# privefl/bigsnpr

Measured on AMD Instinct MI355X. Metric: SNP-cols/sec for bed_randomSVD k=20 (m*passes/wall), higher is better.
Workload: dtype i8 (2-bit codes x 24-bit (early block steps) / 16-bit (late block steps) fixed-point image of the fp64 basis in int8 slices, exact int32 MFMA accumulation; fp64 panel algebra and Rayleigh-Ritz)

## Files before the change

### bigsnpr_amd/_lib.py

```python
import ctypes as C
import os
import threading

import numpy as np

_HERE = os.path.dirname(os.path.abspath(__file__))
LIB_PATH = os.path.join(_HERE, "libbigsnpr_hip.so")

u8p = C.POINTER(C.c_uint8)
i32p = C.POINTER(C.c_int32)
i64p = C.POINTER(C.c_int64)
u64p = C.POINTER(C.c_uint64)
f64p = C.POINTER(C.c_double)
vp = C.c_void_p
i64 = C.c_int64

ALLREDUCE_FN = C.CFUNCTYPE(None, C.c_void_p, C.c_int64, C.c_void_p)


class SvdOptions(C.Structure):
    _fields_ = [("k", C.c_int32), ("tol", C.c_double), ("block", C.c_int32),
                ("slices", C.c_int32), ("max_basis", C.c_int32), ("seed", C.c_uint32),
                ("verbose", C.c_int32), ("m_total", C.c_int64), ("allreduce", ALLREDUCE_FN),
                ("allreduce_ctx", C.c_void_p), ("hook_rank", C.c_int32), ("hook_world", C.c_int32),
# ... 84 lines not shown
    "bsn_bed_project_pca": (C.c_int, [vp, i64p, i64, i64p, i64, f64p, f64p, f64p, i64, f64p, f64p, f64p, f64p]),
    "bsn_project_last_ms": (C.c_int, [f64p]),
    "bsn_mult_lin_reg":(C.c_int, [vp, i64p, i64, i64p, i64, f64p, i64, f64p]),
    "bsn_univ_linreg": (C.c_int, [vp, i64p, i64, i64p, i64, f64p, f64p, i64, f64p, f64p]),
    "bsn_univ_logreg": (C.c_int, [vp, i64p, i64, i64p, i64, f64p, f64p, i64, C.c_double, C.c_int32, f64p, f64p, i32p]),
    "bsn_bed_sp_reg": (C.c_int, [vp, i64p, i64, i64p, i64] + _PLR_TAIL),
    "bsn_dense_sp_reg": (C.c_int, [vp, C.c_int, i64, i64, i64] + _PLR_TAIL),
    "bsn_plr_last_stats": (C.c_int, [f64p]),
    "bsn_impute_simple": (C.c_int, [vp, C.c_int, C.c_uint64, C.POINTER(vp), u8p, i64p]),
    "bsn_impute_last_ms": (C.c_int, [f64p]),
    "bsn_inflate": (C.c_int, [u8p, i64p, i64, u8p, i64p, i32p]),
    "bsn_bgen_read": (C.c_int, [C.c_char_p, i64p, i64, i64, i64p, i64, u8p, C.c_int, C.c_uint64, i64, i64, i64, C.POINTER(vp), u8p,
                                f64p, f64p]),
    "bsn_bgen_prod": (C.c_int, [C.c_char_p, i64p, i64, i64, i64p, i64, f64p, C.c_int, C.c_uint64, i64, f64p, i64, i64, i64, f64p]),
    "bsn_bgen_last_ms": (C.c_int, [f64p]),
    "bsn_bed_group_counts": (C.c_int, [vp, i64p, i64, i32p, C.c_int32, i64p, i64, i32p]),
    "bsn_fst": (C.c_int, [f64p, f64p, i64, i64, C.c_double, f64p, f64p]),
    "bsn_bed_fst": (C.c_int, [vp, i64p, i64, i32p, C.c_int32, i64p, i64, C.c_double, f64p, f64p]),
    "bsn_snp_max3": (C.c_int, [vp, i64p, i64, i32p, i64p, i64, f64p, C.c_int32, f64p]),
    "bsn_popstat_last_ms": (C.c_int, [f64p]),
    "bsn_hwe": (C.c_int, [i32p, i64, C.c_int, f64p]),
    "bsn_hwe_lanes": (C.c_int, [i32p, i64, C.c_int, C.c_int, f64p, f64p]),
    "bsn_bed_hwe": (C.c_int, [vp, i64p, i64, i64p, i64, C.c_int, f64p, i32p]),
    "bsn_bed_qc": (C.c_int, [vp, i64p, i64, i64p, i64, i32p, C.c_double, C.c_double, C.c_double, C.c_double, C.c_int,
                             u8p, u8p, f64p, f64p]),
    "bsn_qc_last_ms": (C.c_int, [f64p]),
    "bsn_bed_king": (C.c_int, [vp, i64p, i64, i64p, i64, C.c_double, C.c_int, C.POINTER(C.c_int64), C.POINTER(vp)]),
    "bsn_king_fetch": (C.c_int, [vp, i32p, i32p, i32p, f64p]),
    "bsn_king_free": (C.c_int, [vp]),
    "bsn_king_last_ms": (C.c_int, [f64p]),
    "bsn_bed_to_fbm": (C.c_int, [vp, i64p, i64, i64p, i64, u8p]),
    "bsn_bed_readbina": (C.c_int, [vp, u8p, u8p]),
    "bsn_bed_is_streamed": (C.c_int, [vp]),
    "bsn_bed_streaming_kernels": (C.c_int, [vp, C.c_char_p, i64]),
    "bsn_bed_subset_payload": (C.c_int, [vp, i64p, i64, i64p, i64, u8p]),
    "bsn_op_create": (C.c_int, [vp, i64p, i64, i64p, i64, f64p, f64p, C.POINTER(vp)]),
    "bsn_op_destroy": (C.c_int, [vp]),
    "bsn_op_set_slices": (C.c_int, [vp, C.c_int]),
    "bsn_op_prod": (C.c_int, [vp, vp, i64, C.c_int, vp, i64]),
    "bsn_op_cprod": (C.c_int, [vp, vp, i64, C.c_int, vp, i64]),
    "bsn_op_sync": (C.c_int, [vp]),
    "bsn_op_last_kernel": (C.c_int, [vp, C.c_char_p, i64]),
    "bsn_bed_randomsvd": (C.c_int, [vp, i64p, i64, i64p, i64, f64p, f64p, C.POINTER(SvdOptions),
                                    f64p, f64p, f64p, C.POINTER(SvdInfo)]),
    "bsn_bed_tcrossprod": (C.c_int, [vp, i64p, i64, i64p, i64, f64p, f64p, i64, f64p]),
    "bsn_cormat": (C.c_int, [vp, i64p, i64, i64p, i64, C.c_double, f64p, f64p, C.c_int, i32p,
                             C.POINTER(C.c_int64), C.POINTER(vp)]),
    "bsn_cormat_fetch": (C.c_int, [vp, i32p, f64p]),
    "bsn_cormat_has_nan": (C.c_int, [vp, C.POINTER(C.c_int)]),
    "bsn_cormat_free": (C.c_int, [vp]),
    "bsn_ld_scores": (C.c_int, [vp, i64p, i64, i64p, i64, C.c_double, f64p, f64p]),
    "bsn_clumping_chr": (C.c_int, [vp, i64p, i64, i64p, i64, C.c_int, f64p, f64p, i32p, i32p, f64p,
                                   C.c_double, C.c_double, i32p]),
    "bsn_clumping_chr_cached": (C.c_int, [vp, i64p, i64, i64p, i64, C.c_int, f64p, f64p, i32p, i32p, f64p,
                                          i64, f64p, f64p, i32p]),
    "bsn_snp_grid_prs": (C.c_int, [vp, i64p, i64, i64p, i64, f64p, i32p, C.POINTER(C.c_uint8), i64, i64,
                                   C.c_int, f64p]),
    "bsn_sfbm_from_csc": (C.c_int, [i64p, i32p, f64p, i64, C.c_int, C.POINTER(vp)]),
    "bsn_sfbm_ncol": (C.c_int, [vp, i64p, i64p, i64p]),
    "bsn_sfbm_free": (C.c_int, [vp]),
    "bsn_lassosum2": (C.c_int, [vp, f64p, i64, f64p, f64p, f64p, i64, i64p, C.c_double, C.c_int32, C.c_double,
                                f64p, i32p, f64p]),
    "bsn_ldpred2_gibbs": (C.c_int, [vp, f64p, f64p, i64, i64p, f64p, f64p, i32p, u64p, i64, C.c_int, C.c_int, C.c_uint64,
                                    f64p, f64p]),
    "bsn_ldpred2_gibbs_sampling": (C.c_int, [vp, f64p, f64p, i64, i64p, C.c_double, C.c_double, C.c_int32, C.c_uint64,
                                             C.c_int, C.c_int, C.c_uint64, f64p, f64p]),
    "bsn_ldpred2_auto": (C.c_int, [vp, f64p, f64p, f64p, i64, i64p, f64p, u64p, i64, C.c_double, C.c_int, C.c_int, C.c_int,
                                   C.c_int, C.c_double, C.c_int, C.c_double, C.c_double, C.c_double, C.c_double,
                                   C.c_double, C.c_uint64, f64p, f64p, f64p, f64p, f64p, f64p, f64p, f64p]),
    "bsn_sfbm_prodvec": (C.c_int, [vp, f64p, i64p, i64, f64p]),
    "bsn_sfbm_ld_scores": (C.c_int, [vp, i64p, i64, f64p]),
    "bsn_sfbm_solve_sym": (C.c_int, [vp, f64p, f64p, i64p, i64, C.c_double, C.c_int32, f64p, i32p, f64p]),
    "bsn_sfbm_last_ms": (C.c_int, [vp, f64p]),
    "bsn_sfbm_ldsplit": (C.c_int, [vp, C.c_double, C.c_double, C.c_int32, C.c_int32, C.c_int32, C.c_double, f64p, f64p, i32p,
                                   f64p, f64p, f64p, i32p, i32p, i32p, f64p]),
    "bsn_panel_gemm_tn": (C.c_int, [vp, i64, C.c_int32, vp, i64, C.c_int32, i64, vp, C.c_int32]),
    "bsn_panel_gemm_nn": (C.c_int, [vp, i64, C.c_int32, vp, C.c_int32, vp, i64, C.c_double, C.c_double, vp, i64, i64]),
    "bsn_panel_right_mult": (C.c_int, [vp, i64, i64, C.c_int32, C.c_int32, vp]),
    "bsn_panel_update": (C.c_int, [vp, i64, C.c_int32, vp, vp, C.c_int32, vp, i64, i64, vp]),
    "bsn_panel_round_cols": (C.c_int, [vp, i64, i64, C.c_int32, C.c_int32, C.c_int32, vp, C.c_int32]),
    "bsn_panel_fused_orth": (C.c_int, [vp, i64, C.c_int32, C.c_int32, C.c_int32, C.c_int32, f64p, f64p]),
    "bsn_panel_compact_gather": (C.c_int, [vp, i64, C.c_int32, C.c_int32, C.c_int32, vp]),
    "bsn_panel_block_roundtrip": (C.c_int, [vp, i64, C.c_int32, C.c_int32, vp, vp]),
    "bsn_malloc": (C.c_int, [C.POINTER(vp), i64]),
    "bsn_free": (C.c_int, [vp]),
    "bsn_host_alloc": (C.c_int, [C.POINTER(vp), i64]),
    "bsn_host_free": (C.c_int, [vp]),
    "bsn_memcpy_h2d": (C.c_int, [vp, vp, i64]),
    "bsn_memcpy_d2h": (C.c_int, [vp, vp, i64]),
    "bsn_device_sync": (C.c_int, []),
    "bsn_timer_start": (C.c_int, [vp]),
    "bsn_timer_stop": (C.c_int, [vp, f64p]),
}

_lib = None


class BsnError(RuntimeError):
    pass


def load():
    global _lib
    if _lib is None:
        LIB_PATH = os.environ.get("BSN_LIB_PATH") or globals()["LIB_PATH"]
        if not os.path.exists(LIB_PATH):
            raise ImportError(
                "%s not found: build it with `python -m bigsnpr_amd.build` "
                "(there is no CPU fallback)" % LIB_PATH)
        lib = C.CDLL(LIB_PATH)
        for name, (res, args) in SIGNATURES.items():
            fn = getattr(lib, name)
            fn.restype = res
            fn.argtypes = args
        _lib = lib
    return _lib


def check(rc):
    if rc != 0:
        raise BsnError(load().bsn_last_error().decode("utf-8", "replace"))


def ptr(a, t):
    return None if a is None else a.ctypes.data_as(t)


def as_i64(a):
    return None if a is None else np.ascontiguousarray(a, dtype=np.int64)


def as_f64(a):
    return None if a is None else np.ascontiguousarray(a, dtype=np.float64)


class DeviceArray:

    def __init__(self, rows, cols=1):
        self.rows, self.cols = int(rows), int(cols)
        p = vp()
        check(load().bsn_malloc(C.byref(p), self.rows * self.cols * 8))
        self.ptr = p

    @classmethod
    def from_numpy(cls, a):
        a = np.asarray(a, dtype=np.float64)
        if a.ndim == 1:
            a = a[:, None]
        d = cls(a.shape[0], a.shape[1])
        h = np.asfortranarray(a)
        check(load().bsn_memcpy_h2d(d.ptr, h.ctypes.data_as(vp), h.nbytes))
        return d

    def to_numpy(self):
        h = np.empty((self.rows, self.cols), dtype=np.float64, order="F")
        check(load().bsn_memcpy_d2h(h.ctypes.data_as(vp), self.ptr, h.nbytes))
        return h

    def col_ptr(self, j):
        return vp(self.ptr.value + 8 * self.rows * j)

    def free(self):
        if self.ptr is not None and self.ptr.value:
            load().bsn_free(self.ptr)
            self.ptr = None

    def __del__(self):
        try:
            self.free()
        except Exception:
            pass


class _PinnedBlock:

    def __init__(self, pool, addr, size):
        self.pool, self.addr, self.size = pool, addr, size
        self.__array_interface__ = {"data": (addr, False), "shape": (size,), "typestr": "|u1", "version": 3}

    def __del__(self):
        try:
            self.pool._give_back(self.addr, self.size)
        except Exception:
            pass


class PinnedPool:

    def __init__(self, keep=None):
        self.free = []
        self.keep = int(os.environ.get("BSN_RESULT_POOL_KEEP", 1 << 30)) if keep is None else keep
        self.keep_max = int(os.environ.get("BSN_RESULT_POOL_MAX", 8 << 30))
        self.live = 0
        self.peak_live = 0
# ... 77 lines not shown
```

### bigsnpr_amd/csrc/matvec.hip

```cpp
#include <cmath>
#include <cstdlib>
#include <map>
#include <mutex>

#include "bsn_internal.hpp"
#include "byte_plan.hpp"
#include "prod_plan.hpp"
#include "prodt_sparse.hpp"
#include <type_traits>

namespace bsn {

typedef int v4i __attribute__((ext_vector_type(4)));
typedef int v8i __attribute__((ext_vector_type(8)));

static thread_local const void *g_last_kernel = nullptr;
#define BSN_KLAUNCH(kern, ...)                 \
  do {                                         \
    g_last_kernel = (const void *)(kern);      \
    hipLaunchKernelGGL(kern, __VA_ARGS__);     \
  } while (0)

__device__ __forceinline__ uint32_t lut4(uint32_t lut, uint32_t sel) {
  return __builtin_amdgcn_perm(lut, lut, sel);
// ... 117 lines not shown
  if (blockIdx.x == 0 && tid == 0) meta[v].qscale = qs;
  double xa[16], xc[16], xs[16];
#pragma unroll
  for (int it = 0; it < 16; it++) {
    const int64_t k = (int64_t)blockIdx.x * 1024 + it * 64 + tid;
    const bool in = k < len;
    xa[it] = in ? X[k + v * ldx] : 0.0;
    xc[it] = 0.0;
    xs[it] = 1.0;
    if (mode == 1) {
      if (in && scale) xs[it] = scale[k];
      if (in && center) xc[it] = center[k];
    } else if (mode == 2) {
      if (in && center) xc[it] = center[k + v * ldx];
    }
  }
#pragma unroll
  for (int it = 0; it < 16; it++) {
    const int t = it * 64 + tid;
    double a = xa[it], b = 0;
    if (mode == 1) {
      a = a / xs[it];
      b = (xc[it] - voff) * a;
      a *= vstep;
    } else if (mode == 2) {
      b = xc[it];
    }
    if (!(fabs(a) <= 1.79e308)) a = 0;
    if (!(fabs(b) <= 1.79e308)) b = 0;
    sa[t + (t >> 4)] = a * qs;
    sb[t + (t >> 4)] = b * qs;
  }
  __syncthreads();
  long long shi = 0, slo = 0, shi2 = 0, slo2 = 0;
  if (kb * 16 < len_pad) {
    uint32_t pk[2][S][4];
#pragma unroll
    for (int p = 0; p < 2; p++)
#pragma unroll
      for (int s = 0; s < S; s++)
#pragma unroll
        for (int w = 0; w < 4; w++) pk[p][s][w] = 0;
#pragma unroll
    for (int e = 0; e < 16; e++) {
      long long A = llrint(sa[tid * 17 + e]), B = llrint(sb[tid * 17 + e]);
      shi += A >> 24; slo += A & 0xFFFFFF;
      shi2 += B >> 24; slo2 += B & 0xFFFFFF;
      if ((raw3 & 1) && PERM != 2) B -= 3 * A;
      const int pos = PERM == 1 ? ((e & 3) * 4 + (e >> 2)) : e;
#pragma unroll
      for (int s = 0; s < S; s++) {
        const int8_t da = (int8_t)(A & 0xFF), db = (int8_t)(B & 0xFF);
        A = (A - da) >> 8;
        B = (B - db) >> 8;
        if constexpr (PERM == 2) {
          const int r = prodt_sparse_row(e), ba = prodt_sparse_byte(e, 0), bb = prodt_sparse_byte(e, 1);
          pk[r][s][ba >> 2] |= (uint32_t)(uint8_t)da << (8 * (ba & 3));
          pk[r][s][bb >> 2] |= (uint32_t)(uint8_t)db << (8 * (bb & 3));
        } else {
          pk[0][s][pos >> 2] |= (uint32_t)(uint8_t)da << (8 * (pos & 3));
          pk[1][s][pos >> 2] |= (uint32_t)(uint8_t)db << (8 * (pos & 3));
        }
      }
    }
    for (int p = 0; p < nplanes; p++)
#pragma unroll
      for (int s = 0; s < S; s++) {
        const int col = v * S + s;
        int8_t *dst = q + ((kb * nplanes + p) * ncol + col) * 16;
        *(uint4 *)dst = p == 0 ? uint4{pk[0][s][0], pk[0][s][1], pk[0][s][2], pk[0][s][3]}
                               : uint4{pk[1][s][0], pk[1][s][1], pk[1][s][2], pk[1][s][3]};
      }
  }
  for (int off = 32; off > 0; off >>= 1) {
    shi += __shfl_down(shi, off); slo += __shfl_down(slo, off);
    shi2 += __shfl_down(shi2, off); slo2 += __shfl_down(slo2, off);
  }
  if (tid == 0) {
    atomicAdd((unsigned long long *)&meta[v].sum_hi, (unsigned long long)shi);
    atomicAdd((unsigned long long *)&meta[v].sum_lo, (unsigned long long)slo);
    if (mode >= 1) {
      atomicAdd((unsigned long long *)&meta[v].sum2_hi, (unsigned long long)shi2);
      atomicAdd((unsigned long long *)&meta[v].sum2_lo, (unsigned long long)slo2);
    }
  }
}

template <int NB, int NPLANE, int KC, bool RAW0, bool STATS, bool CONTIG, int TILES = 2, int WAVES = 8, int MINW = 1,
          int TAG = 0, bool TILED = false, int SGB = 0, bool NASKIP = false>
__global__ __launch_bounds__(64 * WAVES, MINW) void k_cprod(const uint8_t *__restrict__ img, int64_t pitch,
                                               const int32_t *__restrict__ cols, int64_t col0,
                                               int64_t m, const int8_t *__restrict__ xq,
                                               int32_t *__restrict__ acc_out, int64_t m_out,
                                               uint32_t lutA, uint32_t lutB, uint32_t lutC,
                                               int32_t *__restrict__ counts, int32_t n_pad_samples,
                                               const CprodGrid geo, int32_t *__restrict__ part_out) {
  constexpr int NCOL = 16 * NB;
  constexpr int LD = KC / 256;
  constexpr int XS = KC / 16 * NCOL;
  __shared__ uint4 xs[2][XS];
  const int tid = threadIdx.x, wave = tid >> 6, lane = tid & 63;
  const int c = lane & 15, g = lane >> 4;
  constexpr int NT = 64 * WAVES;
  const int nchunks = (int)(pitch * 4 / KC);
  constexpr bool GEO = CONTIG && !TILED && !STATS && NPLANE < 3 && KC == 512;
  CprodSlab sl{(int)blockIdx.x, 0, 0, nchunks};
  if constexpr (GEO) {
    sl = cprod_slab(geo, blockIdx.x);
    sl.block = __builtin_amdgcn_readfirstlane(sl.block), sl.slab = __builtin_amdgcn_readfirstlane(sl.slab);
    sl.ch_begin = __builtin_amdgcn_readfirstlane(sl.ch_begin), sl.ch_end = __builtin_amdgcn_readfirstlane(sl.ch_end);
  }
  const int ch_begin = sl.ch_begin, ch_end = sl.ch_end;
  if (ch_begin >= ch_end) return;
  const int64_t wg_base = (int64_t)sl.block * (WAVES * 16 * TILES);
  const int64_t snp_base = wg_base + wave * (16 * TILES);
  const uint8_t *rowp[TILES];
  uint32_t voff[TILES];
#pragma unroll
  for (int t = 0; t < TILES; t++) {
    int64_t j = snp_base + t * 16 + c;
    if (j > m - 1) j = m - 1;
    int64_t col = CONTIG ? col0 + j : (int64_t)cols[j];
    rowp[t] = img + col * pitch + g * 16;
    voff[t] = TILED ? (uint32_t)((((j - wg_base) >> 6) * (pitch >> 8)) * 16384 + (j & 63) * 256 + g * 16)
                    : (uint32_t)((j - wg_base) * pitch + g * 16);
  }
  static_assert(!TILED || (CONTIG && (WAVES * 16 * TILES) % 64 == 0), "streaming layout: whole 64-variant blocks");
  const __amdgpu_buffer_rsrc_t rs = __builtin_amdgcn_make_buffer_rsrc(
      (void *)(TILED ? img + (((col0 + wg_base) >> 6) * (pitch >> 8)) * 16384
                     : img + (col0 + (CONTIG ? wg_base : 0)) * pitch),
      0, 0x7fffffff, 0x00020000);
  typedef unsigned int v4u __attribute__((ext_vector_type(4)));
  auto gload = [&](const int t, const int off) -> uint4 {
    if constexpr (CONTIG) {
      const int soff = TILED ? ((off >> 8) << 14) + (off & 255) : off;
      const v4u r = __builtin_amdgcn_raw_buffer_load_b128(rs, (int)voff[t], soff, 0);
      return uint4{r.x, r.y, r.z, r.w};
    } else {
      return *(const uint4 *)(rowp[t] + off);
    }
  };
  const uint4 *xq4 = (const uint4 *)xq;

  v4i acc[TILES][NPLANE][NB];
#pragma unroll
  for (int t = 0; t < TILES; t++)
#pragma unroll
    for (int p = 0; p < NPLANE; p++)
#pragma unroll
      for (int nb = 0; nb < NB; nb++) acc[t][p][nb] = v4i{0, 0, 0, 0};
  uint32_t st_lo[TILES], st_hi[TILES], st_na[TILES];
#pragma unroll
  for (int t = 0; t < TILES; t++) st_lo[t] = st_hi[t] = st_na[t] = 0;

  constexpr int NX = (XS + NT - 1) / NT;
  static_assert(NX <= 4, "staging registers");
  constexpr bool XFULL = (XS % NT == 0);
  uint4 ga[2][TILES][LD];
  uint4 xr0 = {0, 0, 0, 0}, xr1 = {0, 0, 0, 0}, xr2 = {0, 0, 0, 0}, xr3 = {0, 0, 0, 0};
#pragma unroll
  for (int t = 0; t < TILES; t++)
#pragma unroll
    for (int it = 0; it < LD; it++) ga[0][t][it] = gload(t, ch_begin * (KC / 4) + it * 64);
  auto staged = [&](const int x) -> bool { return XFULL || tid + x * NT < XS; };
  {
    const uint4 *src = xq4 + (int64_t)ch_begin * XS;
// ... 785 lines not shown
    load(jn2, X[SET]);
#pragma unroll
    for (int q = 0; q < 4; q++) {
      v4i val, na;
      if constexpr (HASNA) {
        uint32_t n0, n1, n2, n3;
        val = v4i{(int)val8m(T[q][0], n0), (int)val8m(T[q][1], n1), (int)val8m(T[q][2], n2), (int)val8m(T[q][3], n3)};
        na = v4i{(int)n0, (int)n1, (int)n2, (int)n3};
      } else {
        val = v4i{(int)T[q][0], (int)T[q][1], (int)T[q][2], (int)T[q][3]};
      }
#pragma unroll
      for (int nb = 0; nb < NB; nb++) {
        acc[q][nb] = __builtin_amdgcn_mfma_i32_16x16x64_i8(aw[nb], val, acc[q][nb], 0, 0, 0);
        if constexpr (HASNA) acc[q][nb] = __builtin_amdgcn_mfma_i32_16x16x64_i8(awc[nb], na, acc[q][nb], 0, 0, 0);
      }
    }
    ws[SET ^ 1][wtid] = wreg;
    __syncthreads();
  };
  for (int64_t jb = j0; jb < j1; jb += 128) {
    step(std::integral_constant<int, 0>{}, jb);
    if (jb + 64 < j1) step(std::integral_constant<int, 1>{}, jb + 64);
  }
  if (wbase < n_pad) {
#pragma unroll
    for (int u = 0; u < 4; u++) {
      const int64_t i = wbase + sg * 4 + u;
#pragma unroll
      for (int nb = 0; nb < NB; nb++)
        *(v4i *)(acc_out + (((int64_t)blockIdx.y * n_pad + i) * NCOL + nb * 16 + 4 * g)) = acc[u][nb];
    }
  }
}

void require_bits(const bsn_bed *b, int bits, const char *what) {
  if (b->bits != bits)
    fail("%s is not available for this handle: it needs %s", what,
         bits == 2 ? "a 2-bit genotype image (.bed, or an FBM.code256 whose codes decode to 0 / 1 / 2 / NA)"
                   : "a byte (dosage) image");
}

void prof_begin(bsn_op *op, int kind, bool more) {
  if (!op->profile) return;
  if (op->prof_kind_override >= 0) kind = op->prof_kind_override;
  op->ev_more.push_back(more);
  hipEvent_t a, b;
  BSN_HIP(hipEventCreate(&a));
  BSN_HIP(hipEventCreate(&b));
  op->ev_begin.push_back(a);
  op->ev_end.push_back(b);
  op->ev_kind.push_back(kind);
  BSN_HIP(hipEventRecord(a, op->bed->stream));
}
void prof_end(bsn_op *op) {
  if (!op->profile) return;
  BSN_HIP(hipEventRecord(op->ev_end.back(), op->bed->stream));
  op->prof_kernel[op->ev_kind.back() % kProfKinds] = g_last_kernel;
}
void prof_collect(bsn_op *op, double ms[kProfKinds], int count[kProfKinds]) {
  for (int k = 0; k < kProfKinds; k++) ms[k] = 0, count[k] = 0;
  for (size_t i = 0; i < op->ev_begin.size(); i++) {
    float t = 0;
    if (hipEventSynchronize(op->ev_end[i]) == hipSuccess &&
        hipEventElapsedTime(&t, op->ev_begin[i], op->ev_end[i]) == hipSuccess) {
      ms[op->ev_kind[i]] += t;
      if (!op->ev_more[i]) count[op->ev_kind[i]]++;
    }
    (void)hipEventDestroy(op->ev_begin[i]);
    (void)hipEventDestroy(op->ev_end[i]);
  }
  (void)hipGetLastError();
  op->ev_begin.clear();
  op->ev_end.clear();
  op->ev_kind.clear();
  op->ev_more.clear();
}

static VecMeta *meta_buffer(bsn_op *op) {
  return (VecMeta *)op->d_meta.ensure((size_t)kMetaVecs * 8 + (size_t)kMetaVecs * 256 * 2);
}
static inline int64_t n_padded(const bsn_bed *b) { return b->bits == 8 ? b->pitch : b->pitch * 4; }

static void quantise(bsn_op *op, const double *d_X, int64_t ldx, int64_t len, int64_t len_pad,
                     int nvec, int mode, int S, int ncol, int permute, int exact_int,
                     VecMeta *meta, int8_t *q, const double *d_W2 = nullptr) {
  hipStream_t st = op->bed->stream;
  const bool bytes = op->bed->bits == 8;
  const double vstep = bytes ? op->bed->v_step : 1.0, voff = bytes ? op->bed->v_off : 0.0;
  const int raw3 = (!bytes && mode == 1) ? 1 : 0;
  if (bytes) permute = 0;
  if (permute == 2 && !(mode == 1 && (raw3 & 1))) fail("internal: the interleaved digit rows are the scaled product's");
  double *part = (double *)(meta + kMetaVecs);
  int gx = 0;
  if (exact_int) {
    hipLaunchKernelGGL(k_meta_clear, dim3(1), dim3(64), 0, st, meta, nvec);
  } else {
    gx = (int)((len + 1023) / 1024);
    if (gx > 256) gx = 256;
    hipLaunchKernelGGL(k_absmax, dim3(gx, nvec), dim3(1024), 0, st, d_X, ldx, len,
                       mode == 1 ? op->d_center.p : mode == 2 ? d_W2 : nullptr,
                       mode == 1 ? op->d_scale.p : nullptr, mode, meta, part, vstep, voff, raw3);
  }
  int64_t nblk = len_pad / 16;
  const double *qc = mode == 1 ? op->d_center.p : mode == 2 ? d_W2 : nullptr;
  const double *qsc = mode == 1 ? op->d_scale.p : nullptr;
  const dim3 qgrid((unsigned)((nblk + 63) / 64), nvec);
#define BSN_QUANT(SV)                                                                                  \
  case SV:                                                                                             \
    if (permute == 2)                                                                                  \
      hipLaunchKernelGGL((k_quant<SV, 2>), qgrid, dim3(64), 0, st, d_X, ldx, len, len_pad, qc, qsc, mode, \
                         ncol, meta, q, vstep, voff, raw3, part, gx);                                  \
    else if (permute)                                                                                  \
      hipLaunchKernelGGL((k_quant<SV, 1>), qgrid, dim3(64), 0, st, d_X, ldx, len, len_pad, qc, qsc, mode, \
                         ncol, meta, q, vstep, voff, raw3, part, gx);                                  \
    else                                                                                               \
      hipLaunchKernelGGL((k_quant<SV, 0>), qgrid, dim3(64), 0, st, d_X, ldx, len, len_pad, qc, qsc, mode, \
                         ncol, meta, q, vstep, voff, raw3, part, gx);                                  \
    break;
  switch (S) {
    BSN_QUANT(1) BSN_QUANT(2) BSN_QUANT(3) BSN_QUANT(4) BSN_QUANT(5) BSN_QUANT(6) BSN_QUANT(7) BSN_QUANT(8)
    default: fail("slices must be in 1..8");
  }
#undef BSN_QUANT
  BSN_HIP(hipGetLastError());
}

static const double *scatter_rows_if_needed(bsn_op *op, const double *d_X, int64_t *ldx,
                                            int nvec) {
  if (op->rows_identity) return d_X;
  bsn_bed *b = op->bed;
  double *xf = op->d_xfull.ensure((size_t)b->n * nvec);
  BSN_HIP(hipMemsetAsync(xf, 0, (size_t)b->n * nvec * sizeof(double), b->stream));
  hipLaunchKernelGGL(k_scatter_rows, dim3((unsigned)((op->n + 255) / 256), nvec), dim3(256), 0,
                     b->stream, d_X, *ldx, op->d_rows.p, op->n, xf, b->n);
  BSN_HIP(hipGetLastError());
  *ldx = b->n;
  return xf;
}

#pragma clang fp contract(off)
__global__ void k_binom_scale(const int32_t *counts, int64_t m, double *center, double *scale) {
  int64_t j = (int64_t)blockIdx.x * blockDim.x + threadIdx.x;
  if (j >= m) return;
  const int4 c = *(const int4 *)(counts + 4 * j);
  const double sumX = (double)(c.y + 2 * c.z);
  const double nona = (double)(c.x + c.y + c.z);
  const double af = sumX / (2.0 * nona);
  center[j] = 2.0 * af;
  scale[j] = sqrt(2.0 * af * (1.0 - af));
}
#pragma clang fp contract(on)

__global__ __launch_bounds__(256) void k_stats_summary(const int32_t *counts, int64_t m, int64_t n, int32_t *na,
                                                       unsigned long long *out) {
  long long s = 0, bad = 0;
  for (int64_t j = (int64_t)blockIdx.x * 256 + threadIdx.x; j < m; j += (int64_t)gridDim.x * 256) {
    const int4 c = *(const int4 *)(counts + 4 * j);
    s += c.w;
    na[j] = c.w;
    if (2 * ((int64_t)c.x + c.y + c.z) < n) bad++;
  }
  for (int off = 32; off > 0; off >>= 1) {
    s += __shfl_down(s, off);
    bad += __shfl_down(bad, off);
  }
  __shared__ long long sw[4], sb[4];
  if ((threadIdx.x & 63) == 0) {
    sw[threadIdx.x >> 6] = s;
    sb[threadIdx.x >> 6] = bad;
  }
  __syncthreads();
  if (threadIdx.x == 0) {
    s = sw[0] + sw[1] + sw[2] + sw[3];
    bad = sb[0] + sb[1] + sb[2] + sb[3];
    if (s) atomicAdd(&out[0], (unsigned long long)s);
    if (bad) atomicAdd(&out[1], (unsigned long long)bad);
  }
}

static bool use_tiled(const bsn_op *op) {
  return op->bed->d_tiled != nullptr && op->cols_contig && (op->col0 & 63) == 0;
}

static int device_cus() {
  static const int ncu = [] {
    hipDeviceProp_t pr;
    int dev = 0;
    return (hipGetDevice(&dev) == hipSuccess && hipGetDeviceProperties(&pr, dev) == hipSuccess && pr.multiProcessorCount > 0)
               ? pr.multiProcessorCount : 256;
  }();
  return ncu;
}

static thread_local CprodGridFacts g_cprod_facts;
static CprodGrid cprod_geometry(bsn_op *op, const void *kern, int per_wg, int threads, int NB, int nplane) {
  static std::mutex mu;
  static std::map<const void *, int> held;
  int resident;
  {
    std::lock_guard<std::mutex> lk(mu);
    auto it = held.find(kern);
    if (it == held.end()) {
      int nb = 0;
      if (hipOccupancyMaxActiveBlocksPerMultiprocessor(&nb, kern, threads, 0) != hipSuccess || nb < 1) nb = 1;
      it = held.emplace(kern, nb).first;
    }
    resident = it->second;
  }
  CprodGridFacts f;
  f.m = op->m, f.per_wg = per_wg, f.nchunks = (int)(op->bed->pitch * 4 / 512), f.pitch = op->bed->pitch;
  f.NB = NB, f.nplane = nplane, f.ncu = device_cus(), f.resident = resident;
  if (const char *e = getenv("BSN_PLAN_CUS")) f.ncu = std::max(1, atoi(e));
  if (const char *e = getenv("BSN_CPROD_SLABS")) f.slabs = std::max(1, atoi(e));
  g_cprod_facts = f;
  return plan_cprod(f);
}

template <int NPLANE, bool RAW0, bool STATS>
static void launch_cprod(bsn_op *op, int NB, const int8_t *q, int32_t *acc, uint32_t l0,
                         uint32_t l1, uint32_t l2, int32_t *counts = nullptr, CprodGrid *geo = nullptr,
                         int32_t *part = nullptr) {
  bsn_bed *b = op->bed;
  constexpr int KC = 512, TT = STATS ? 2 : 4;
  constexpr bool PLAIN = NPLANE == 2 && RAW0 && !STATS;
  if (b->pitch * 4 > 4000000) fail("more than 4e6 samples are not supported by the crossproduct kernel");
  const int32_t *cols = op->cols_contig ? nullptr : op->d_cols.p;
  const int32_t npad = (int32_t)(b->pitch * 4 - b->n);
  CprodFacts f;
  f.NB = NB, f.plain = PLAIN, f.stats = STATS, f.cols_contig = op->cols_contig, f.tiled = use_tiled(op);
  f.warm = op->prof_kind_override == 3, f.na_skip = op->na_skip_c;
  const CprodKernel k = choose_cprod(f);
  const uint8_t *image = k.tiled ? b->d_tiled : b->d_img;
  const int per_wg = 16 * k.tiles * k.waves;
  const bool geo_ok = geo && k.contig && !k.tiled && !STATS && NPLANE < 3 && !getenv("BSN_CPROD_ONE_SPLIT");
  CprodGrid one;
  one.blocks = one.blocks_whole = (int)((op->m + per_wg - 1) / per_wg), one.nchunks = (int)(b->pitch * 4 / KC);
  const bool planning = geo && !acc;
  if (planning && !geo_ok) {
    *geo = one;
    return;
  }
  const CprodGrid g = geo && !planning ? *geo : one;
  const dim3 grid((unsigned)cprod_workgroups(g)), block(64 * k.waves);
#define BSN_CPROD(NBV, CONTIGV, TV, WV, TAGV, TILEDV, SGBV, NASKIPV)                                                   \
  if (k == CprodKernel{NBV, CONTIGV, TV, WV, TAGV, TILEDV, SGBV, NASKIPV}) {                                           \
    auto kern = k_cprod<NBV, NPLANE, KC, RAW0, STATS, CONTIGV, TV, WV, 1, TAGV, TILEDV, SGBV, NASKIPV>;                \
    if (planning) {                                                                                                    \
      *geo = cprod_geometry(op, (const void *)kern, per_wg, 64 * k.waves, NB, NPLANE);                                 \
      return;                                                                                                          \
    }                                                                                                                  \
    BSN_KLAUNCH(kern, grid, block, 0, b->stream, image, b->pitch, cols, op->col0, op->m, q, acc, op->m, l0, l1, l2,    \
                counts, npad, g, part);                                                                                \
    BSN_HIP(hipGetLastError());                                                                                        \
    return;                                                                                                            \
  }
  BSN_CPROD(1, false, 2, 8, 0, false, 0, false)
  BSN_CPROD(1, true, 2, 8, 0, false, 0, false)
  BSN_CPROD(1, true, 2, 8, 1, false, 0, false)
  BSN_CPROD(1, true, TT, 8, 0, true, 0, false)
  BSN_CPROD(1, true, TT, 8, 1, true, 0, false)
  BSN_CPROD(2, false, 2, 16, 0, false, 0, false)
  BSN_CPROD(2, true, 2, 16, 0, false, 3, false)
  BSN_CPROD(2, true, 2, 16, 0, true, 3, false)
  if constexpr (!STATS && NPLANE < 3) {
    BSN_CPROD(3, false, 2, 16, 0, false, 0, false)
    BSN_CPROD(3, true, 2, 16, 0, false, 3, false)
  }
  if constexpr (PLAIN) {
    BSN_CPROD(2, false, 2, 16, 0, false, 0, true)
    BSN_CPROD(2, true, 2, 16, 0, false, 0, true)
    BSN_CPROD(3, false, 2, 16, 0, false, 0, true)
    BSN_CPROD(3, true, 2, 16, 0, false, 0, true)
  }
#undef BSN_CPROD
// ... 558 lines not shown
                    bool one_digit, int32_t *d_table, double ms_out[3]) {
  require_bits(op->bed, 2, "bed_counts_by_group");
  op->preq_X = nullptr;
  bsn_bed *b = op->bed;
  hipStream_t st = b->stream;
  const int S = one_digit ? 1 : 4, per_block = 16 / S;
  const int64_t npad = n_padded(b), nblk = npad / 16;
  const int gmax = G < 2 * per_block ? G : 2 * per_block;
  DevBuf<int32_t> mult;
  mult.ensure((size_t)b->n * gmax);
  int8_t *q = op->d_q.ensure((size_t)npad * 32);
  int32_t *acc = op->d_acc.ensure((size_t)3 * op->m * 32);
  std::unique_ptr<EventMarks<4>> ev(ms_out ? new EventMarks<4>() : nullptr);
  for (int g0 = 0; g0 < G;) {
    const int left = G - g0;
    const int NB = left > per_block ? 2 : 1;
    const int gb = left < NB * per_block ? left : NB * per_block, ncol = 16 * NB;
    if (ev) ev->mark(0, st);
    BSN_HIP(hipMemsetAsync(mult.p, 0, (size_t)b->n * gb * sizeof(int32_t), st));
    hipLaunchKernelGGL(k_group_scatter, dim3((unsigned)((n + 255) / 256)), dim3(256), 0, st, d_rows, d_group, n, g0, gb,
                       b->n, mult.p);
    const dim3 qgrid((unsigned)((nblk + 255) / 256), (unsigned)gb);
    if (S == 1) hipLaunchKernelGGL(k_group_digits<1>, qgrid, dim3(256), 0, st, mult.p, b->n, nblk, gb, ncol, q);
    else hipLaunchKernelGGL(k_group_digits<4>, qgrid, dim3(256), 0, st, mult.p, b->n, nblk, gb, ncol, q);
    BSN_HIP(hipGetLastError());
    if (ev) ev->mark(1, st);
    launch_cprod<3, false, false>(op, NB, q, acc, kLutHom2, kLutHet, kLutNA);
    if (ev) ev->mark(2, st);
    hipLaunchKernelGGL(k_group_counts_final, dim3((unsigned)((op->m * gb + 255) / 256)), dim3(256), 0, st, acc, op->m, ncol,
                       S, g0, gb, G, d_gsize, d_table);
    BSN_HIP(hipGetLastError());
    if (ev) {
      ev->mark(3, st);
      BSN_HIP(hipEventSynchronize(ev->e[3]));
      for (int k = 0; k < 3; k++) ms_out[k] += ev->ms(k, k + 1);
    }
    g0 += gb;
  }
  BSN_HIP(hipStreamSynchronize(st));
}

__global__ void k_selftest(int *out) {
  int lane = threadIdx.x;
  uint32_t r = perm8(0x77665544u, 0x33221100u, 0x07040300u);
  int ok_perm = (r == 0x77443300u);
  v4i a = {0, 0, 0, 0}, b = {0, 0, 0, 0};
  int i = lane & 15, gq = lane >> 4;
  for (int e = 0; e < 16; e++) {
    int k = gq * 16 + e;
    int av = (k == (5 * i + 3) % 64) ? (i + 1) : 0;
    int bv = (k % 7) - 3 + i;
    a[e >> 2] |= (av & 0xFF) << (8 * (e & 3));
    b[e >> 2] |= (bv & 0xFF) << (8 * (e & 3));
  }
  v4i c = {0, 0, 0, 0};
  c = __builtin_amdgcn_mfma_i32_16x16x64_i8(a, b, c, 0, 0, 0);
  int ok_mfma = 1;
  for (int rr = 0; rr < 4; rr++) {
    int row = 4 * gq + rr, col = lane & 15;
    int k = (5 * row + 3) % 64;
    int want = (row + 1) * ((k % 7) - 3 + col);
    if (c[rr] != want) ok_mfma = 0;
  }
  int all_perm = __all(ok_perm), all_mfma = __all(ok_mfma);
  if (lane == 0) {
    out[0] = all_perm;
    out[1] = all_mfma;
    out[2] = (int)r;
  }
}

void selftest() {
  DevBuf<int> d;
  d.ensure(4);
  hipLaunchKernelGGL(k_selftest, dim3(1), dim3(64), 0, 0, d.p);
  BSN_HIP(hipGetLastError());
  int h[4] = {0, 0, 0, 0};
  BSN_HIP(hipMemcpy(h, d.p, sizeof(h), hipMemcpyDeviceToHost));
  if (!h[0]) fail("selftest: v_perm_b32 byte order differs from the assumed {hi:lo} (got %08x)", h[2]);
  if (!h[1]) fail("selftest: v_mfma_i32_16x16x64_i8 operand/accumulator layout differs");
}

}
```

### include/bigsnpr_hip.h

```cpp
#ifndef BIGSNPR_HIP_H
#define BIGSNPR_HIP_H

#include <stdint.h>

#ifdef __cplusplus
extern "C" {
#endif

typedef struct bsn_bed bsn_bed;
typedef struct bsn_op bsn_op;

const char *bsn_last_error(void);
int bsn_version(void);
int bsn_device_count(int *count);
int bsn_set_device(int device);
int bsn_selftest(void);

int bsn_bed_open(const char *path, int64_t n, int64_t m, bsn_bed **out);
int bsn_bed_is_streamed(const bsn_bed *bed);
int bsn_bed_from_host(const uint8_t *payload, int64_t n, int64_t m, int64_t n_byte, bsn_bed **out);
int bsn_bed_from_fbm(const uint8_t *bytes, int64_t n, int64_t m, int64_t ld, bsn_bed **out);
int bsn_fbm_open(const uint8_t *bytes, int64_t n, int64_t m, int64_t ld, const double *code256, bsn_bed **out);
int bsn_bed_bits(const bsn_bed *bed);
int64_t bsn_bed_na_known(const bsn_bed *bed);
// ... 218 lines not shown
int bsn_bed_tcrossprod(bsn_bed *bed, const int64_t *ind_row, int64_t n, const int64_t *ind_col,
                       int64_t m, const double *center, const double *scale, int64_t block_size,
                       double *K);

typedef struct bsn_cor bsn_cor;
int bsn_cormat(bsn_bed *bed, const int64_t *ind_row, int64_t n, const int64_t *ind_col, int64_t m,
               double size, const double *thr, const double *pos, int fill_diag, int32_t *p_out,
               int64_t *nnz_out, bsn_cor **out);
int bsn_cormat_fetch(bsn_cor *cor, int32_t *i_out, double *x_out);
int bsn_cormat_has_nan(const bsn_cor *cor, int *out);
int bsn_cormat_free(bsn_cor *cor);
int bsn_ld_last_stats(double *out );
int bsn_ld_scores(bsn_bed *bed, const int64_t *ind_row, int64_t n, const int64_t *ind_col, int64_t m,
                  double size, const double *pos, double *out);
int bsn_clumping_chr(bsn_bed *bed, const int64_t *ind_row, int64_t n, const int64_t *ind_col,
                     int64_t m, int mode, const double *aux1, const double *aux2,
                     const int32_t *ordInd, const int32_t *rankInd, const double *pos, double size,
                     double thr, int32_t *keep);
int bsn_clumping_chr_cached(bsn_bed *bed, const int64_t *ind_row, int64_t n, const int64_t *ind_col,
                            int64_t m, int mode, const double *aux1, const double *aux2,
                            const int32_t *ordInd, const int32_t *rankInd, const double *pos,
                            int64_t n_grid, const double *sizes, const double *thrs, int32_t *keep);

int bsn_robust_scale_tau2(const double *d_X, int64_t m, int64_t ld, int32_t ncol, double c1, double c2, double *mu_out, double *s_out);
int bsn_robust_medians(const double *d_X, int64_t m, int64_t ld, int32_t ncol, const double *centre, double *med_out);
int bsn_robust_pair_scales(const double *d_Z, int64_t m, int64_t ld, int32_t p, double c1, double c2, double *s_sum_out, double *s_diff_out);
int bsn_robust_mc_count(const double *d_up, int64_t nu, const double *d_lo, int64_t nl, double t, int64_t *count_out);
int bsn_robust_scale_cols(double *d_Z, int64_t m, int64_t ld, int32_t p, const double *div );
int bsn_robust_rotate(double *d_Z, int64_t m, int64_t ld, int32_t p, const double *E );
int bsn_robust_wdist(const double *d_Z, int64_t m, int64_t ld, int32_t p, const double *mu, const double *sig, double *out);
int bsn_robust_dist_ogk(const double *d_U, int64_t m, int64_t ld, int32_t p, int32_t niter, double cut_ratio, double c1, double c2,
                        double *dist_out, int64_t *n_kept_out);
int bsn_robust_rollmean(const double *x, int64_t m, const double *w, int32_t len, const int64_t *group_off, int32_t ngroups, double *out);
int bsn_robust_sort(double *x, int64_t m);
int bsn_robust_mc_window(const double *d_up, int64_t nu, const double *d_lo, int64_t nl, double a, double b, int64_t cap, double *out,
                         int64_t *count_out);

int bsn_order_decreasing(const double *S, int64_t m, const int64_t *group_off, int32_t ngroups, int32_t *ord, int32_t *rank);

typedef struct bsn_sfbm bsn_sfbm;
int bsn_sfbm_from_csc(const int64_t *p, const int32_t *i, const double *x, int64_t m2, int upper, bsn_sfbm **out);
int bsn_sfbm_ncol(const bsn_sfbm *s, int64_t *m2_out, int64_t *nnz_out, int64_t *bandwidth_out);
int bsn_sfbm_free(bsn_sfbm *s);
int bsn_lassosum2(const bsn_sfbm *s, const double *beta_hat, int64_t m, const double *pf, const double *lambda,
                  const double *delta, int64_t G, const int64_t *ind_sub, double dfmax, int32_t maxiter, double tol,
                  double *beta_out, int32_t *num_iter_out, double *time_out);
int bsn_ldpred2_gibbs(const bsn_sfbm *s, const double *beta_hat, const double *n_vec, int64_t m, const int64_t *ind_sub,
                      const double *h2, const double *p, const int32_t *sparse, const uint64_t *stream, int64_t G, int burn_in,
                      int num_iter, uint64_t seed, double *beta_out, double *seconds_out);
int bsn_ldpred2_gibbs_sampling(const bsn_sfbm *s, const double *beta_hat, const double *n_vec, int64_t m, const int64_t *ind_sub,
                               double h2, double p, int32_t sparse, uint64_t stream, int burn_in, int num_iter, uint64_t seed,
                               double *sample_out, double *seconds_out);
int bsn_ldpred2_auto(const bsn_sfbm *s, const double *beta_hat, const double *n_vec, const double *log_var, int64_t m,
                     const int64_t *ind_sub, const double *p_init, const uint64_t *stream, int64_t G, double h2_init,
                     int burn_in, int num_iter, int report_step, int no_jump_sign, double shrink_corr, int use_mle,
                     double p_lo, double p_hi, double alpha_lo, double alpha_hi, double mean_ld, uint64_t seed,
                     double *beta_est, double *postp_est, double *corr_est, double *sample_beta,
                     double *path_p, double *path_h2, double *path_alpha, double *seconds_out);

int bsn_sfbm_prodvec(bsn_sfbm *s, const double *x, const int64_t *ind_sub, int64_t m, double *y_out);
int bsn_sfbm_ld_scores(bsn_sfbm *s, const int64_t *ind_sub, int64_t m, double *out);
int bsn_sfbm_solve_sym(bsn_sfbm *s, const double *b, const double *add_to_diag, const int64_t *ind_sub, int64_t m, double tol,
                       int32_t maxiter, double *x_out, int32_t *iters_out, double *relres_out);
int bsn_sfbm_last_ms(const bsn_sfbm *s, double *ms_out);

int bsn_sfbm_ldsplit(const bsn_sfbm *s, double thr_r2, double max_r2, int32_t min_size, int32_t max_size, int32_t max_K,
                     double max_cost, const double *pos_scaled, double *C_out, int32_t *best_ind_out, double *cost_out,
                     double *cost2_out, double *perc_kept_out, int32_t *n_block_ok_out, int32_t *all_last_out,
                     int32_t *levels_run_out, double *seconds_out);

int bsn_panel_gemm_tn(const double *d_A, int64_t lda, int32_t p, const double *d_B, int64_t ldb, int32_t cb, int64_t rows,
                      double *d_C, int32_t ldc);
int bsn_panel_gemm_nn(const double *d_Q, int64_t ldq, int32_t p, const double *d_S, int32_t nc, const double *d_In, int64_t ldi,
                      double alpha, double beta, double *d_Out, int64_t ldo, int64_t n);
int bsn_panel_right_mult(double *d_W, int64_t ld, int64_t n, int32_t cb, int32_t r, const double *d_M);
int bsn_panel_update(const double *d_Q, int64_t ldq, int32_t p, const double *d_C, const double *d_Ri, int32_t cb, double *d_W,
                     int64_t ldw, int64_t n, uint64_t *d_mx);
int bsn_panel_round_cols(double *d_X, int64_t ld, int64_t rows, int32_t cb, int32_t slices, int32_t have_mx, uint64_t *d_mx,
                         int32_t wide_grid);
int bsn_panel_fused_orth(double *d_QW, int64_t nr, int32_t p, int32_t p0, int32_t cb, int32_t iters, double *flag_out,
                         double *Rout_out);
int bsn_panel_compact_gather(const double *d_full, int64_t n, int32_t cb, int32_t world, int32_t slices, double *d_out);
int bsn_panel_block_roundtrip(const double *d_full, int64_t n, int32_t cb, int32_t world, double *d_out, double *d_placed);

int bsn_malloc(void **d_ptr, int64_t bytes);
int bsn_free(void *d_ptr);
int bsn_host_alloc(void **h_ptr, int64_t bytes);
int bsn_host_free(void *h_ptr);
int bsn_memcpy_h2d(void *d_dst, const void *src, int64_t bytes);
int bsn_memcpy_d2h(void *dst, const void *d_src, int64_t bytes);
int bsn_device_sync(void);
int bsn_timer_start(bsn_bed *bed);
int bsn_timer_stop(bsn_bed *bed, double *ms);

#ifdef __cplusplus
}
#endif
#endif
```

Before: 39.43 million.

## Quantise whole basis panel in one tiled kernel instead of per-vector grids

```diff
diff --git a/bigsnpr_amd/_lib.py b/bigsnpr_amd/_lib.py
--- a/bigsnpr_amd/_lib.py
+++ b/bigsnpr_amd/_lib.py
@@ -190,6 +190,8 @@
     "bsn_panel_fused_orth": (C.c_int, [vp, i64, C.c_int32, C.c_int32, C.c_int32, C.c_int32, f64p, f64p]),
     "bsn_panel_compact_gather": (C.c_int, [vp, i64, C.c_int32, C.c_int32, C.c_int32, vp]),
     "bsn_panel_block_roundtrip": (C.c_int, [vp, i64, C.c_int32, C.c_int32, vp, vp]),
+    "bsn_quant_panel": (C.c_int, [vp, i64, i64, i64, C.c_int32, C.c_int32, C.c_int32, C.c_int32, C.c_int32, vp, vp, C.c_int32,
+                                  C.c_int32, vp, vp]),
     "bsn_malloc": (C.c_int, [C.POINTER(vp), i64]),
     "bsn_free": (C.c_int, [vp]),
     "bsn_host_alloc": (C.c_int, [C.POINTER(vp), i64]),
@@ -218,6 +220,8 @@
                 "(there is no CPU fallback)" % LIB_PATH)
         lib = C.CDLL(LIB_PATH)
         for name, (res, args) in SIGNATURES.items():
+            if name == "bsn_quant_panel" and not hasattr(lib, name):
+                continue
             fn = getattr(lib, name)
             fn.restype = res
             fn.argtypes = args
diff --git a/bigsnpr_amd/csrc/matvec.hip b/bigsnpr_amd/csrc/matvec.hip
--- a/bigsnpr_amd/csrc/matvec.hip
+++ b/bigsnpr_amd/csrc/matvec.hip
@@ -223,6 +223,154 @@
     if (mode >= 1) {
       atomicAdd((unsigned long long *)&meta[v].sum2_hi, (unsigned long long)shi2);
       atomicAdd((unsigned long long *)&meta[v].sum2_lo, (unsigned long long)slo2);
+    }
+  }
+}
+
+constexpr int kQuantTileBlocks = 16;
+constexpr int kQuantTileK = 16 * kQuantTileBlocks;
+constexpr int kQuantPanelVecs = 16;
+template <int S, int PERM>
+__global__ __launch_bounds__(kQuantTileK) void k_quant_panel(const double *__restrict__ X, int64_t ldx, int64_t len,
+                                                             int64_t len_pad, const double *__restrict__ center,
+                                                             const double *__restrict__ scale, int mode, int ncol,
+                                                             int nvec, int tiles, VecMeta *meta, int8_t *__restrict__ q,
+                                                             double vstep, double voff, int raw3,
+                                                             const double *__restrict__ part, int gx) {
+  static_assert(S >= 1 && S <= 3, "the staged integers are int32");
+  constexpr int NT = kQuantTileK, LDW = 17;
+  static_assert(2 * NT * LDW * 4 >= kQuantTileBlocks * 2 * kMaxCols * 16, "the digit rows of a tile fit the value staging");
+  __shared__ uint4 lds4[2 * NT * LDW * 4 / 16];
+  __shared__ double s_qs[kQuantPanelVecs];
+  __shared__ long long s_sum[NT / 64][kQuantPanelVecs][4];
+  int32_t *const sa = (int32_t *)lds4, *const sb = sa + NT * LDW;
+  const int tid = threadIdx.x, wave = tid >> 6, lane = tid & 63;
+  const int nplanes = mode >= 1 ? 2 : 1, nused = nvec * S;
+  for (int v = wave; v < nvec; v += NT / 64) {
+    double mx = 0, bad = 0;
+    for (int t = lane; t < gx; t += 64) {
+      mx = fmax(mx, part[((int64_t)v * gx + t) * 2]);
+      bad += part[((int64_t)v * gx + t) * 2 + 1];
+    }
+    for (int off = 32; off > 0; off >>= 1) {
+      mx = fmax(mx, __shfl_xor(mx, off));
+      bad += __shfl_xor(bad, off);
+    }
+    double qs = 0.0;
+    if (mx > 0) {
+      int e;
+      frexp(ldexp(0.99, 8 * S - 1) / mx, &e);
+      qs = ldexp(1.0, e - 1);
+    }
+    if (lane == 0) {
+      s_qs[v] = qs;
+      if (blockIdx.x == 0) {
+        meta[v].absmax_bits = (unsigned long long)__double_as_longlong(mx);
+        meta[v].nonfinite = (unsigned long long)bad;
+        meta[v].qscale = qs;
+      }
+    }
+  }
+  __syncthreads();
+  const int v2 = tid & 15, kbl = tid >> 4;
+  long long shi = 0, slo = 0, shi2 = 0, slo2 = 0;
+  for (int tile = 0; tile < tiles; tile++) {
+    const int64_t kb0 = ((int64_t)blockIdx.x * tiles + tile) * kQuantTileBlocks;
+    if (kb0 * 16 >= len_pad) break;
+    const int64_t k = kb0 * 16 + tid;
+    const bool in = k < len;
+    double xs = 1.0, xc = 0.0, xa[kQuantPanelVecs];
+    if (mode == 1) {
+      if (in && scale) xs = scale[k];
+      if (in && center) xc = center[k];
+    }
+#pragma unroll
+    for (int v = 0; v < kQuantPanelVecs; v++) xa[v] = (in && v < nvec) ? X[k + v * ldx] : 0.0;
+#pragma unroll
+    for (int v = 0; v < kQuantPanelVecs; v++) {
+      if (v < nvec) {
+        double a = xa[v], b = 0;
+        if (mode == 1) {
+          a = a / xs;
+          b = (xc - voff) * a;
+          a *= vstep;
+        }
+        if (!(fabs(a) <= 1.79e308)) a = 0;
+        if (!(fabs(b) <= 1.79e308)) b = 0;
+        const double qs = s_qs[v];
+        sa[tid * LDW + v] = (int32_t)llrint(a * qs);
+        sb[tid * LDW + v] = (int32_t)llrint(b * qs);
+      }
+    }
+    __syncthreads();
+    uint32_t pk[2][S][4];
+#pragma unroll
+    for (int p = 0; p < 2; p++)
+#pragma unroll
+      for (int s = 0; s < S; s++)
+#pragma unroll
+        for (int w = 0; w < 4; w++) pk[p][s][w] = 0;
+    if (v2 < nvec) {
+#pragma unroll
+      for (int e = 0; e < 16; e++) {
+        long long A = sa[(kbl * 16 + e) * LDW + v2], B = sb[(kbl * 16 + e) * LDW + v2];
+        shi += A >> 24; slo += A & 0xFFFFFF;
+        shi2 += B >> 24; slo2 += B & 0xFFFFFF;
+        if ((raw3 & 1) && PERM != 2) B -= 3 * A;
+        const int pos = PERM == 1 ? ((e & 3) * 4 + (e >> 2)) : e;
+#pragma unroll
+        for (int s = 0; s < S; s++) {
+          const int8_t da = (int8_t)(A & 0xFF), db = (int8_t)(B & 0xFF);
+          A = (A - da) >> 8;
+          B = (B - db) >> 8;
+          if constexpr (PERM == 2) {
+            const int r = prodt_sparse_row(e), ba = prodt_sparse_byte(e, 0), bb = prodt_sparse_byte(e, 1);
+            pk[r][s][ba >> 2] |= (uint32_t)(uint8_t)da << (8 * (ba & 3));
+            pk[r][s][bb >> 2] |= (uint32_t)(uint8_t)db << (8 * (bb & 3));
+          } else {
+            pk[0][s][pos >> 2] |= (uint32_t)(uint8_t)da << (8 * (pos & 3));
+            pk[1][s][pos >> 2] |= (uint32_t)(uint8_t)db << (8 * (pos & 3));
+          }
+        }
+      }
+    }
+    __syncthreads();
+    if (v2 < nvec) {
+      for (int p = 0; p < nplanes; p++)
+#pragma unroll
+        for (int s = 0; s < S; s++)
+          lds4[(kbl * nplanes + p) * nused + v2 * S + s] =
+              p == 0 ? uint4{pk[0][s][0], pk[0][s][1], pk[0][s][2], pk[0][s][3]}
+                     : uint4{pk[1][s][0], pk[1][s][1], pk[1][s][2], pk[1][s][3]};
+    }
+    __syncthreads();
+    int64_t nb = len_pad / 16 - kb0;
+    if (nb > kQuantTileBlocks) nb = kQuantTileBlocks;
+    const int nrows = (int)nb * nplanes * nused;
+    uint4 *const qrow = (uint4 *)q + kb0 * nplanes * ncol;
+    for (int u = tid; u < nrows; u += NT) {
+      const int run = u / nused, c = u - run * nused;
+      qrow[(int64_t)run * ncol + c] = lds4[u];
+    }
+    __syncthreads();
+  }
+  for (int off = 32; off >= 16; off >>= 1) {
+    shi += __shfl_xor(shi, off); slo += __shfl_xor(slo, off);
+    shi2 += __shfl_xor(shi2, off); slo2 += __shfl_xor(slo2, off);
+  }
+  if (lane < 16) {
+    s_sum[wave][lane][0] = shi; s_sum[wave][lane][1] = slo;
+    s_sum[wave][lane][2] = shi2; s_sum[wave][lane][3] = slo2;
+  }
+  __syncthreads();
+  if (tid < 64) {
+    const int v = tid >> 2, w = tid & 3;
+    if (v < nvec && (w < 2 || mode >= 1)) {
+      long long s = 0;
+      for (int i = 0; i < NT / 64; i++) s += s_sum[i][v][w];
+      unsigned long long *dst = (unsigned long long *)(w == 0 ? &meta[v].sum_hi : w == 1 ? &meta[v].sum_lo
+                                                      : w == 2 ? &meta[v].sum2_hi : &meta[v].sum2_lo);
+      atomicAdd(dst, (unsigned long long)s);
     }
   }
 }
@@ -1174,29 +1322,59 @@
 }
 static inline int64_t n_padded(const bsn_bed *b) { return b->bits == 8 ? b->pitch : b->pitch * 4; }
 
-static void quantise(bsn_op *op, const double *d_X, int64_t ldx, int64_t len, int64_t len_pad,
-                     int nvec, int mode, int S, int ncol, int permute, int exact_int,
-                     VecMeta *meta, int8_t *q, const double *d_W2 = nullptr) {
-  hipStream_t st = op->bed->stream;
-  const bool bytes = op->bed->bits == 8;
-  const double vstep = bytes ? op->bed->v_step : 1.0, voff = bytes ? op->bed->v_off : 0.0;
-  const int raw3 = (!bytes && mode == 1) ? 1 : 0;
-  if (bytes) permute = 0;
+static int device_cus() {
+  static const int ncu = [] {
+    hipDeviceProp_t pr;
+    int dev = 0;
+    return (hipGetDevice(&dev) == hipSuccess && hipGetDeviceProperties(&pr, dev) == hipSuccess && pr.multiProcessorCount > 0)
+               ? pr.multiProcessorCount : 256;
+  }();
+  return ncu;
+}
+
+static void quantise_on(hipStream_t st, bool two_bit, double vstep, double voff, const double *d_center, const double *d_scale,
+                        const double *d_X, int64_t ldx, int64_t len, int64_t len_pad, int nvec, int mode, int S, int ncol,
+                        int permute, int exact_int, VecMeta *meta, int8_t *q, const double *d_W2, bool per_vector, int tiles) {
+  const int raw3 = (two_bit && mode == 1) ? 1 : 0;
+  if (!two_bit) permute = 0;
   if (permute == 2 && !(mode == 1 && (raw3 & 1))) fail("internal: the interleaved digit rows are the scaled product's");
   double *part = (double *)(meta + kMetaVecs);
   int gx = 0;
+  const double *qc = mode == 1 ? d_center : mode == 2 ? d_W2 : nullptr;
+  const double *qsc = mode == 1 ? d_scale : nullptr;
   if (exact_int) {
     hipLaunchKernelGGL(k_meta_clear, dim3(1), dim3(64), 0, st, meta, nvec);
   } else {
     gx = (int)((len + 1023) / 1024);
     if (gx > 256) gx = 256;
-    hipLaunchKernelGGL(k_absmax, dim3(gx, nvec), dim3(1024), 0, st, d_X, ldx, len,
-                       mode == 1 ? op->d_center.p : mode == 2 ? d_W2 : nullptr,
-                       mode == 1 ? op->d_scale.p : nullptr, mode, meta, part, vstep, voff, raw3);
+    hipLaunchKernelGGL(k_absmax, dim3(gx, nvec), dim3(1024), 0, st, d_X, ldx, len, qc, qsc, mode, meta, part, vstep, voff,
+                       raw3);
   }
   int64_t nblk = len_pad / 16;
-  const double *qc = mode == 1 ? op->d_center.p : mode == 2 ? d_W2 : nullptr;
-  const double *qsc = mode == 1 ? op->d_scale.p : nullptr;
+  if (two_bit && !exact_int && mode <= 1 && nvec <= kQuantPanelVecs && S >= 1 && S <= 3 && nvec * S <= ncol && ncol <= kMaxCols &&
+      !per_vector && !getenv("BSN_QUANT_PER_VECTOR")) {
+    const int64_t ntiles = (nblk + kQuantTileBlocks - 1) / kQuantTileBlocks;
+    const int64_t places = 3 * (int64_t)device_cus();
+    if (tiles <= 0) tiles = (int)std::max<int64_t>(1, std::min<int64_t>(8, (ntiles + places - 1) / places));
+    const dim3 pgrid((unsigned)((ntiles + tiles - 1) / tiles));
+#define BSN_QUANT_PANEL(SV, PV)                                                                                  \
+  hipLaunchKernelGGL((k_quant_panel<SV, PV>), pgrid, dim3(kQuantTileK), 0, st, d_X, ldx, len, len_pad, qc, qsc, mode, ncol, \
+                     nvec, tiles, meta, q, vstep, voff, raw3, part, gx)
+#define BSN_QUANT_PANEL_S(SV)                      \
+  case SV:                                         \
+    if (permute == 2) BSN_QUANT_PANEL(SV, 2);      \
+    else if (permute) BSN_QUANT_PANEL(SV, 1);      \
+    else BSN_QUANT_PANEL(SV, 0);                   \
+    break;
+    switch (S) {
+      BSN_QUANT_PANEL_S(1) BSN_QUANT_PANEL_S(2) BSN_QUANT_PANEL_S(3)
+      default: fail("slices must be in 1..8");
+    }
+#undef BSN_QUANT_PANEL_S
+#undef BSN_QUANT_PANEL
+    BSN_HIP(hipGetLastError());
+    return;
+  }
   const dim3 qgrid((unsigned)((nblk + 63) / 64), nvec);
 #define BSN_QUANT(SV)                                                                                  \
   case SV:                                                                                             \
@@ -1218,6 +1396,15 @@
   BSN_HIP(hipGetLastError());
 }
 
+static void quantise(bsn_op *op, const double *d_X, int64_t ldx, int64_t len, int64_t len_pad,
+                     int nvec, int mode, int S, int ncol, int permute, int exact_int,
+                     VecMeta *meta, int8_t *q, const double *d_W2 = nullptr) {
+  const bsn_bed *b = op->bed;
+  const bool bytes = b->bits == 8;
+  quantise_on(b->stream, !bytes, bytes ? b->v_step : 1.0, bytes ? b->v_off : 0.0, op->d_center.p, op->d_scale.p, d_X, ldx, len,
+              len_pad, nvec, mode, S, ncol, permute, exact_int, meta, q, d_W2, false, 0);
+}
+
 static const double *scatter_rows_if_needed(bsn_op *op, const double *d_X, int64_t *ldx,
                                             int nvec) {
   if (op->rows_identity) return d_X;
@@ -1273,16 +1460,6 @@
 
 static bool use_tiled(const bsn_op *op) {
   return op->bed->d_tiled != nullptr && op->cols_contig && (op->col0 & 63) == 0;
-}
-
-static int device_cus() {
-  static const int ncu = [] {
-    hipDeviceProp_t pr;
-    int dev = 0;
-    return (hipGetDevice(&dev) == hipSuccess && hipGetDeviceProperties(&pr, dev) == hipSuccess && pr.multiProcessorCount > 0)
-               ? pr.multiProcessorCount : 256;
-  }();
-  return ncu;
 }
 
 static thread_local CprodGridFacts g_cprod_facts;
@@ -2007,3 +2184,25 @@
 }
 
 }
+
+extern "C" int bsn_quant_panel(const double *d_X, int64_t ldx, int64_t len, int64_t len_pad, int32_t nvec, int32_t mode,
+                               int32_t slices, int32_t ncol, int32_t perm, const double *d_center, const double *d_scale,
+                               int32_t per_vector, int32_t tiles, void *d_meta, int8_t *d_q) {
+  using namespace bsn;
+  return guarded([&] {
+    require_gpu();
+    if (!d_X || !d_meta || !d_q) fail("bsn_quant_panel: null pointer");
+    if (mode < 0 || mode > 1 || perm < 0 || perm > 2 || (perm == 2 && mode != 1))
+      fail("bsn_quant_panel: mode 0 or 1, byte order 0, 1 or 2 (2 with mode 1 only)");
+    if (len < 1 || len > ((int64_t)1 << 31) || len_pad < len || len_pad % 16 != 0 || len_pad > ((int64_t)1 << 31) || ldx < len ||
+        nvec < 1 || nvec > kQuantPanelVecs || slices < 1 || slices > 3 || (ncol != 16 && ncol != 32 && ncol != 48) ||
+        nvec * slices > ncol || tiles < 0 || tiles > 64)
+      fail("bsn_quant_panel: dimensions (at most %d vectors of 1 to 3 slices in 16, 32 or 48 columns)", kQuantPanelVecs);
+    DevBuf<double> work;
+    VecMeta *meta = (VecMeta *)work.ensure((size_t)kMetaVecs * 8 + (size_t)kMetaVecs * 256 * 2);
+    quantise_on(nullptr, true, 1.0, 0.0, d_center, d_scale, d_X, ldx, len, len_pad, nvec, mode, slices, ncol, perm, 0, meta, d_q,
+                nullptr, per_vector != 0, tiles);
+    BSN_HIP(hipMemcpyAsync(d_meta, meta, (size_t)nvec * sizeof(VecMeta), hipMemcpyDeviceToDevice, nullptr));
+    BSN_HIP(hipStreamSynchronize(nullptr));
+  });
+}
diff --git a/include/bigsnpr_hip.h b/include/bigsnpr_hip.h
--- a/include/bigsnpr_hip.h
+++ b/include/bigsnpr_hip.h
@@ -324,6 +324,9 @@
                          double *Rout_out);
 int bsn_panel_compact_gather(const double *d_full, int64_t n, int32_t cb, int32_t world, int32_t slices, double *d_out);
 int bsn_panel_block_roundtrip(const double *d_full, int64_t n, int32_t cb, int32_t world, double *d_out, double *d_placed);
+int bsn_quant_panel(const double *d_X, int64_t ldx, int64_t len, int64_t len_pad, int32_t nvec, int32_t mode, int32_t slices,
+                    int32_t ncol, int32_t perm, const double *d_center, const double *d_scale, int32_t per_vector, int32_t tiles,
+                    void *d_meta, int8_t *d_q);
 
 int bsn_malloc(void **d_ptr, int64_t bytes);
 int bsn_free(void *d_ptr);
```

Measured after the change: 39.61 million, median of 6. No clear change (+0.5%).
